# microsoft/VidTok

Hardware: AMD Instinct MI355X
Metric: encode+decode frames/sec, vidtok_kl_causal_488_4chn 17x256x256 (higher is better)
Workload: dtype bf16; 1 GPU; vidtok_kl_causal_488_4chn forward (encode+KL+decode), bf16, B=4 clips/GPU, 17x256x256; global_batch=4, launch=hipGraph replay (engine graph cache)

## Files before the change

vidtok_amd/csrc/options.cpp:

```cpp
#include "options.h"

#include <stdlib.h>
#include <string.h>

#include <atomic>
#include <mutex>

#include "../../include/vidtok_amd.h"

void vt_set_error(const char* fmt, ...);

namespace {
struct OptDef {
  const char* name;
  int dflt;
};
const OptDef kDefs[OPT_COUNT] = {
    {"conv_buf", 1},        {"conv_tinner", 1},     {"conv_ldsepi", 1},      {"conv_ws", 2},
    {"conv_narrow", 1},     {"conv_tile", 0},       {"conv_tile_min", 128},  {"conv_fuse_ln", 1}, {"conv_fuse_ln256", 1},
    {"tblock_fused", 1},    {"tblock_prof_mode", 0},
    {"conv_deep", 1},       {"ws_prof_mode", 0},    {"attn_flash", 1},      {"conv_splitk", 1},
    {"conv_tskip", 1},      {"conv_in8", 1},        {"conv_tup_ln", 1},     {"conv_nt_mb", 64},
};
std::atomic<int> g_val[OPT_COUNT];
std::once_flag g_once;

int env_default(int id) {
  char var[64] = "VT_";
  size_t n = 3;
  for (const char* s = kDefs[id].name; *s && n + 1 < sizeof(var); ++s) var[n++] = (*s >= 'a' && *s <= 'z') ? (char)(*s - 32) : *s;
  var[n] = 0;
  const char* e = getenv(var);
  return e ? atoi(e) : kDefs[id].dflt;
}
void init_all() {
  for (int i = 0; i < OPT_COUNT; ++i) g_val[i].store(env_default(i), std::memory_order_relaxed);
}
int find(const char* name) {
  if (!name) return -1;
  for (int i = 0; i < OPT_COUNT; ++i)
    if (strcmp(name, kDefs[i].name) == 0) return i;
  return -1;
}
}

int vt_opt(int id) {
  std::call_once(g_once, init_all);
  return g_val[id].load(std::memory_order_relaxed);
}

extern "C" int vt_set_option(const char* name, int32_t value) {
  const int id = find(name);
  if (id < 0) {
    vt_set_error("vt_set_option: unknown option '%s'", name ? name : "(null)");
    return VT_ERR_ARG;
  }
  std::call_once(g_once, init_all);
  g_val[id].store(value, std::memory_order_relaxed);
  return VT_OK;
}

extern "C" int vt_get_option(const char* name, int32_t* value) {
  const int id = find(name);
  if (id < 0 || !value) {
    vt_set_error("vt_get_option: unknown option '%s' or null output", name ? name : "(null)");
    return VT_ERR_ARG;
  }
  *value = vt_opt(id);
  return VT_OK;
}

extern "C" int vt_reset_options(void) {
  std::call_once(g_once, init_all);
  init_all();
  return VT_OK;
}

extern "C" int vt_option_count(void) { return OPT_COUNT; }
extern "C" const char* vt_option_name(int32_t i) { return (i >= 0 && i < OPT_COUNT) ? kDefs[i].name : nullptr; }
```

vidtok_amd/csrc/options.h:

```cpp
#pragma once

enum VtOpt {
  OPT_CONV_BUF = 0,
  OPT_CONV_TINNER,
  OPT_CONV_LDSEPI,
  OPT_CONV_WS,
  OPT_CONV_NARROW,
  OPT_CONV_TILE,
  OPT_CONV_TILE_MIN,
  OPT_CONV_FUSE_LN,
  OPT_CONV_FUSE_LN256,
  OPT_TBLOCK_FUSED,
  OPT_TBLOCK_PROF_MODE,
  OPT_CONV_DEEP,
  OPT_WS_PROF_MODE,
  OPT_ATTN_FLASH,
  OPT_CONV_SPLITK,
  OPT_CONV_TSKIP,
  OPT_CONV_IN8,
  OPT_CONV_TUP_LN,
  OPT_CONV_NT_MB,
  OPT_COUNT
};

int vt_opt(int id);
```

vidtok_amd/csrc/tblock_ws128.hip:

```cpp
#include <atomic>
#include <type_traits>

#include "conv_common.h"

#define VT_STORE_AUX 2

namespace {

[[maybe_unused]] constexpr int TB_PIX = 64;
[[maybe_unused]] constexpr int TB_ROWP = 272;
[[maybe_unused]] constexpr int TB_SLOT = TB_PIX * TB_ROWP;
[[maybe_unused]] constexpr int TB_RING = 3 * TB_SLOT;
[[maybe_unused]] constexpr int TB_T = TB_PIX * 128 * 4;

typedef uint16_t tb_h;
struct TBlockArgs {
  const tb_h* x;
  tb_h* y;
  tb_h* n_out;
  const tb_h* w1;
  const tb_h* w2;
  const float* b1;
  const float* b2;
  const float* g1; const float* be1;
  const float* g2; const float* be2;
  const float* gn; const float* ben;
  int B, T, HW;
  int replicate;
  tb_h* cache1;
  tb_h* cache2;
  int cache_off;
  int keep_y;
  int ln_next;
  float eps;
  unsigned long long* prof;
  int prof_mode;
};

template <int I, int N, typename F>
__device__ __forceinline__ void tb_static_for(F&& f) {
  if constexpr (I < N) {
    f(std::integral_constant<int, I>{});
    tb_static_for<I + 1, N>(f);
  }
}

#pragma clang fp contract(off)
typedef float f32x2 __attribute__((ext_vector_type(2)));
template <typename H>
__device__ __forceinline__ uint32_t tb_pack2(f32x2 v) {
  return h16<H>::pack(v[0], v[1]);
}

[[maybe_unused]] constexpr int T3_T1P = 256;
[[maybe_unused]] constexpr int T3_OFF_T1 = 2 * TB_RING;
[[maybe_unused]] constexpr int T3_OFF_T2 = 2 * TB_RING + TB_PIX * T3_T1P;
[[maybe_unused]] constexpr int T3_LDS = T3_OFF_T2 + TB_T;
template <typename H>
__device__ __forceinline__ void t3_unpack8(const u32x4& w, float (&v)[8]) {
#pragma unroll
  for (int q = 0; q < 4; ++q) {
    v[2 * q] = h16<H>::lo(w[q]);
    v[2 * q + 1] = h16<H>::hi(w[q]);
  }
}
template <typename H>
__device__ __forceinline__ u32x4 t3_pack8(const float (&o)[8]) {
  u32x4 w;
#pragma unroll
  for (int q = 0; q < 4; ++q) w[q] = tb_pack2<H>(f32x2{o[2 * q], o[2 * q + 1]});
  return w;
}

[[maybe_unused]] constexpr int T4_OFF_PRM = T3_LDS;
[[maybe_unused]] constexpr int T4_LDS = T4_OFF_PRM + 8 * 128 * 4;
[[maybe_unused]] constexpr int T4_FD = 6;

template <typename H, bool FIRST>
__device__ __forceinline__ void t4_mfma(const u32x4& w, const u32x4& x, f32x16& acc) {
  if constexpr (std::is_same<H, bf16_t>::value) {
    if constexpr (FIRST) asm volatile("v_mfma_f32_32x32x16_bf16 %0, %1, %2, 0" : "=v"(acc) : "a"(w), "v"(x));
    else asm volatile("v_mfma_f32_32x32x16_bf16 %0, %1, %2, %0" : "+v"(acc) : "a"(w), "v"(x));
  } else {
    if constexpr (FIRST) asm volatile("v_mfma_f32_32x32x16_f16 %0, %1, %2, 0" : "=v"(acc) : "a"(w), "v"(x));
    else asm volatile("v_mfma_f32_32x32x16_f16 %0, %1, %2, %0" : "+v"(acc) : "a"(w), "v"(x));
  }
}
template <bool SILU>
__device__ __forceinline__ void t4_row_norm(float (&v)[8], const float (&g)[8], const float (&b)[8], float eps, float (&o)[8]) {
  ln_row8<16, SILU>(v, g, b, eps, o);
}

template <typename H, int LNN, bool KEEP, bool CACHE, bool PROF = false>
__global__ __launch_bounds__(512, 1) void tblock_pair_kernel(const TBlockArgs p) {
#if defined(__HIP_DEVICE_COMPILE__)
  extern __shared__ __attribute__((aligned(16))) char smem[];
  const int tid = threadIdx.x;
  const int lane = tid & 63;
  const int wave = __builtin_amdgcn_readfirstlane(tid >> 6);
  const int cw = wave & 3, grp = wave >> 2;
  const int ptiles = p.HW / TB_PIX;
  const int ncols = p.B * ptiles;
  const int G = gridDim.x;
  const int slot_id = xcd_remap(blockIdx.x, G);
  const int cq = ncols / G, cr = ncols - cq * G;
  const int c_begin = slot_id * cq + min(slot_id, cr);
  const int c_end = c_begin + cq + (slot_id < cr ? 1 : 0);
  if (c_begin >= c_end) return;
  if (grp == 1) __builtin_amdgcn_s_setprio(2);
  const int n = (c_end - c_begin) * p.T;
  constexpr int R1 = 0, R2 = TB_RING;
  const unsigned frame_bytes = (unsigned)p.HW * 256u;

  float* prm = reinterpret_cast<float*>(smem + T4_OFF_PRM);
  {
    const int c = tid & 127, a = tid >> 7;
    const int pc = ((c >> 2) & 1) * 64 + (c >> 3) * 4 + (c & 3);
    const float* src0 = a == 0 ? p.g1 : (a == 1 ? p.be1 : (a == 2 ? p.g2 : p.be2));
    prm[a * 128 + pc] = ln_fold(src0[c], true);
    float v;
    if (a == 0) v = LNN ? ln_fold(p.gn[c], LNN == 2) : 1.0f;
    else if (a == 1) v = LNN ? ln_fold(p.ben[c], LNN == 2) : 0.0f;
    else if (a == 2) v = p.b1 ? p.b1[c] : 0.0f;
    else v = p.b2 ? p.b2[c] : 0.0f;
    prm[(a + 4) * 128 + pc] = v;
  }

  struct Cur {
    int b, pt, t;
  };
  auto cur_at = [&](int k) __attribute__((always_inline)) {
    Cur c;
    const int q = k / p.T;
    c.t = k - q * p.T;
    const int col = c_begin + q;
    c.b = col / ptiles;
    c.pt = col - c.b * ptiles;
    return c;
  };
  auto cur_step = [&](Cur& c) __attribute__((always_inline)) {
    c.t += 1;
    if (c.t == p.T) {
      c.t = 0;
      c.pt += 1;
      if (c.pt == ptiles) {
        c.pt = 0;
        c.b += 1;
      }
    }
  };
  auto frame_rsrc = [&](const tb_h* base, const Cur& c) __attribute__((always_inline)) {
    return __builtin_amdgcn_make_buffer_rsrc(const_cast<tb_h*>(base) + ((long long)c.b * p.T + c.t) * p.HW * 128, 0, frame_bytes, 0x00020000);
  };

  unsigned long long* stamps = reinterpret_cast<unsigned long long*>(smem + T4_LDS);
  int kcur = 0;
  auto stamp = [&](int i) __attribute__((always_inline)) {
    if constexpr (PROF) {
      if (blockIdx.x == 0 && kcur >= 8 && kcur < 12) {
        const unsigned long long ts = __builtin_amdgcn_s_memtime();
        if (lane == 0) stamps[((kcur - 8) * 8 + wave) * 8 + i] = ts;
      }
    }
  };
  auto dump = [&]() __attribute__((always_inline)) {
    if constexpr (PROF) {
      if (blockIdx.x == 0 && lane == 0)
        for (int i = 0; i < 32; ++i) p.prof[wave * 32 + i] = stamps[((i / 8) * 8 + wave) * 8 + (i % 8)];
    }
  };

  u32x4 wreg[24];
  {
    const tb_h* wsrc = grp == 0 ? p.w1 : p.w2;
    const long long roff = (long long)(cw * 32 + (lane & 31)) * 384 + (lane >> 5) * 8;
#pragma unroll
    for (int g = 0; g < 24; ++g) wreg[g] = *reinterpret_cast<const u32x4*>(wsrc + roff + g * 16);
    __builtin_amdgcn_s_waitcnt(0x0F70);
  }
  f32x16 acc[2];
  auto gemm = [&](auto kt0_c, int roff, int s3, int t) __attribute__((always_inline)) {
    constexpr int KT0 = decltype(kt0_c)::value;
    constexpr int M0 = 16 * KT0;
    int lo = lane;
    asm volatile("" : "+v"(lo));
    const int frag_off = roff + (lo & 31) * TB_ROWP + (lo >> 5) * 16;
    int sp[3];
#pragma unroll
    for (int kt = 0; kt < 3; ++kt) {
      const int back = (t - 2 + kt >= 0 || (CACHE && p.replicate == 2)) ? 2 - kt : t;
      int sl = s3 - back;
      sl = sl < 0 ? sl + 3 : sl;
      sp[kt] = frag_off + sl * TB_SLOT;
    }
    auto faddr = [&](int m) __attribute__((always_inline)) -> const u32x4* {
      const int g = m >> 1, j = m & 1;
      return reinterpret_cast<const u32x4*>(smem + sp[g >> 3] + j * (32 * TB_ROWP) + (g & 7) * 32);
    };
    u32x4 xf[T4_FD + 1];
#pragma unroll
    for (int m = M0; m < M0 + T4_FD; ++m) xf[m % (T4_FD + 1)] = *faddr(m);
    if (grp == 1) __builtin_amdgcn_s_setprio(3);
    tb_static_for<M0, 48>([&](auto mc) __attribute__((always_inline)) {
      constexpr int m = decltype(mc)::value;
      t4_mfma<H, (m < M0 + 2)>(wreg[m >> 1], xf[m % (T4_FD + 1)], acc[m & 1]);
      if constexpr (m + T4_FD < 48) xf[(m + T4_FD) % (T4_FD + 1)] = *faddr(m + T4_FD);
      __builtin_amdgcn_sched_barrier(0);
    });
    if (grp == 1) __builtin_amdgcn_s_setprio(2);
    asm volatile("s_nop 15\n\ts_nop 3" ::: "memory");
  };
  auto run_gemm = [&](int roff, int s3, int t) __attribute__((always_inline)) {
    const int first = p.replicate != 0 ? 0 : max(0, 2 - t);
    if (first == 0) gemm(std::integral_constant<int, 0>{}, roff, s3, t);
    else if (first == 1) gemm(std::integral_constant<int, 1>{}, roff, s3, t);
    else gemm(std::integral_constant<int, 2>{}, roff, s3, t);
  };
  auto acc_to_T1 = [&]() __attribute__((always_inline)) {
    int lo = lane;
    asm volatile("" : "+v"(lo));
    const int l31 = lo & 31;
    const int base = T3_OFF_T1 + l31 * T3_T1P + 8 * (lo >> 5);
#pragma unroll
    for (int j = 0; j < 2; ++j)
#pragma unroll
      for (int g = 0; g < 4; ++g) {
        u32x2 w;
        w[0] = tb_pack2<H>(f32x2{acc[j][4 * g], acc[j][4 * g + 1]});
        w[1] = tb_pack2<H>(f32x2{acc[j][4 * g + 2], acc[j][4 * g + 3]});
        *reinterpret_cast<u32x2*>(smem + base + j * (32 * T3_T1P) + (((4 * cw + g) ^ (l31 & 15)) << 4)) = w;
      }
  };
  auto acc_to_T2 = [&]() __attribute__((always_inline)) {
    int lo = lane;
    asm volatile("" : "+v"(lo));
    const int l31 = lo & 31;
    const int base = T3_OFF_T2 + l31 * 512 + (((cw * 8 + (lo >> 5)) ^ l31) << 4);
#pragma unroll
    for (int j = 0; j < 2; ++j)
#pragma unroll
      for (int g = 0; g < 4; ++g) {
        f32x4 v;
#pragma unroll
        for (int e = 0; e < 4; ++e) v[e] = acc[j][4 * g + e];
        *reinterpret_cast<f32x4*>(smem + ((base ^ (g << 5)) + j * (32 * 512))) = v;
      }
  };

  auto unit_geom = [&](int& oct_j, int& row0) __attribute__((always_inline)) {
    int tt = tid;
    asm volatile("" : "+v"(tt));
    const int vt = tt & 255;
    oct_j = vt & 15;
    row0 = vt >> 4;
  };
  auto ld_prm = [&](int arr, int oct_j, float (&o)[8]) __attribute__((always_inline)) {
    const f32x4 a = *reinterpret_cast<const f32x4*>(prm + arr * 128 + 4 * oct_j);
    const f32x4 b = *reinterpret_cast<const f32x4*>(prm + arr * 128 + 64 + 4 * oct_j);
#pragma unroll
    for (int e = 0; e < 4; ++e) {
      o[e] = a[e];
      o[4 + e] = b[e];
    }
  };
  auto load_rows = [&](auto u0_c, auto u1_c, u32x4 (&dst)[4], const Cur& c) __attribute__((always_inline)) {
    constexpr int U0 = decltype(u0_c)::value, U1 = decltype(u1_c)::value;
    int oct_j, row0;
    unit_geom(oct_j, row0);
    const __amdgpu_buffer_rsrc_t rs = frame_rsrc(p.x, c);
    const int vo = (c.pt * TB_PIX + row0) * 256 + oct_j * 16;
#pragma unroll
    for (int it = U0; it < U1; ++it) dst[it] = __builtin_amdgcn_raw_buffer_load_b128(rs, vo + it * (16 * 256), 0, 0);
  };
  auto cache_put = [&](tb_h* cache, const Cur& c, int oct_j, int row, const u32x4& w) __attribute__((always_inline)) {
    if constexpr (!CACHE) return;
    const int j = c.t - (p.T - p.cache_off - 2);
    if (cache != nullptr && (j == 0 || j == 1)) {
      const __amdgpu_buffer_rsrc_t rs = __builtin_amdgcn_make_buffer_rsrc(cache + ((long long)c.b * 2 + j) * p.HW * 128, 0, frame_bytes, 0x00020000);
      __builtin_amdgcn_raw_buffer_store_b128(w, rs, (c.pt * TB_PIX + row) * 256 + oct_j * 16, 0, 0);
    }
  };
  auto cache_get = [&](const tb_h* cache, int roff, const Cur& c, int sl2, int sl1) __attribute__((always_inline)) {
    if constexpr (!CACHE) return;
    int oct_j, row0;
    unit_geom(oct_j, row0);
    u32x4 w[2][4];
#pragma unroll
    for (int j = 0; j < 2; ++j) {
      const __amdgpu_buffer_rsrc_t rs = __builtin_amdgcn_make_buffer_rsrc(const_cast<tb_h*>(cache) + ((long long)c.b * 2 + j) * p.HW * 128, 0, frame_bytes, 0x00020000);
#pragma unroll
      for (int it = 0; it < 4; ++it) w[j][it] = __builtin_amdgcn_raw_buffer_load_b128(rs, (c.pt * TB_PIX + row0 + 16 * it) * 256 + oct_j * 16, 0, 0);
    }
#pragma unroll
    for (int j = 0; j < 2; ++j)
#pragma unroll
      for (int it = 0; it < 4; ++it)
        *reinterpret_cast<u32x4*>(smem + roff + (j == 0 ? sl2 : sl1) * TB_SLOT + (row0 + 16 * it) * TB_ROWP + oct_j * 16) = w[j][it];
  };
  auto ln1_units = [&](auto u0_c, auto u1_c, const u32x4 (&xr)[4], int s3, const Cur& c) __attribute__((always_inline)) {
    constexpr int U0 = decltype(u0_c)::value, U1 = decltype(u1_c)::value;
    int oct_j, row0;
    unit_geom(oct_j, row0);
    float g[8], b[8];
    ld_prm(0, oct_j, g);
    ld_prm(1, oct_j, b);
    const int wo = R1 + s3 * TB_SLOT + row0 * TB_ROWP + oct_j * 16;
#pragma unroll
    for (int it = U0; it < U1; ++it) {
      float v[8], o[8];
      t3_unpack8<H>(xr[it], v);
      t4_row_norm<true>(v, g, b, p.eps, o);
      const u32x4 w = t3_pack8<H>(o);
      *reinterpret_cast<u32x4*>(smem + wo + it * (16 * TB_ROWP)) = w;
      cache_put(p.cache1, c, oct_j, row0 + 16 * it, w);
      __builtin_amdgcn_sched_barrier(0);
    }
  };

  auto out_store = [&](const u32x4& w, __amdgpu_buffer_rsrc_t rs, int vo) __attribute__((always_inline)) {
    if constexpr (PROF) {
      if (p.prof_mode & 16) return;
    }
    __builtin_amdgcn_raw_buffer_store_b128(w, rs, vo, 0, VT_STORE_AUX);
  };
  struct XSet {
    u32x4 xn[4], xr[4];
  };
  XSet xs;
  Cur c_p2 = cur_at(0);
  Cur c_p1 = c_p2, c_0 = c_p2, c_m1 = c_p2, c_m2 = c_p2;
  __syncthreads();
  constexpr int L1G0 = 3;
  using IL = std::integral_constant<int, L1G0>;
  if (grp == 0) {
    load_rows(std::integral_constant<int, 0>{}, IL{}, xs.xn, c_0);
    ln1_units(std::integral_constant<int, 0>{}, IL{}, xs.xn, 0, c_0);
  } else {
    load_rows(IL{}, std::integral_constant<int, 4>{}, xs.xn, c_0);
    ln1_units(IL{}, std::integral_constant<int, 4>{}, xs.xn, 0, c_0);
    if (CACHE && p.replicate == 2) cache_get(p.cache1, R1, c_0, 1, 2);
  }
  cur_step(c_p1);
  c_p2 = c_p1;
  cur_step(c_p2);
  if (1 < n) {
    if (grp == 0) load_rows(std::integral_constant<int, 0>{}, IL{}, xs.xn, c_p1);
    else load_rows(IL{}, std::integral_constant<int, 4>{}, xs.xn, c_p1);
  }
  if (grp == 0) {
#pragma unroll
    for (int it = 0; it < 2; ++it) xs.xr[it] = xs.xn[0];
  } else {
#pragma unroll
    for (int it = 2; it < 4; ++it) xs.xr[it] = xs.xn[3];
  }
  int s3 = 0;
  auto advance = [&]() __attribute__((always_inline)) {
    c_m2 = c_m1;
    c_m1 = c_0;
    c_0 = c_p1;
    c_p1 = c_p2;
    cur_step(c_p2);
    s3 = s3 == 2 ? 0 : s3 + 1;
  };
  auto slot_back = [&](int back) __attribute__((always_inline)) {
    const int s = s3 - back;
    return s < 0 ? s + 3 : s;
  };
  __syncthreads();

  auto l2_units = [&](auto u0_c, auto u1_c, int sl, const Cur& c) __attribute__((always_inline)) {
    constexpr int U0 = decltype(u0_c)::value, U1 = decltype(u1_c)::value;
    int oct_j, row0;
    unit_geom(oct_j, row0);
    float bo1[8], g[8], b[8];
    ld_prm(6, oct_j, bo1);
    ld_prm(2, oct_j, g);
    ld_prm(3, oct_j, b);
    const int ro = T3_OFF_T1 + row0 * T3_T1P + ((oct_j ^ row0) << 4);
    const int wo = R2 + sl * TB_SLOT + row0 * TB_ROWP + oct_j * 16;
    u32x4 tw[4];
    tw[U0] = *reinterpret_cast<const u32x4*>(smem + ro + U0 * (16 * T3_T1P));
#pragma unroll
    for (int it = U0; it < U1; ++it) {
      if (it + 1 < U1) tw[it + 1] = *reinterpret_cast<const u32x4*>(smem + ro + (it + 1) * (16 * T3_T1P));
      float v[8], o[8];
      t3_unpack8<H>(tw[it], v);
#pragma unroll
      for (int e = 0; e < 8; ++e) v[e] = v[e] + bo1[e];
      t4_row_norm<true>(v, g, b, p.eps, o);
      const u32x4 w = t3_pack8<H>(o);
      *reinterpret_cast<u32x4*>(smem + wo + it * (16 * TB_ROWP)) = w;
      cache_put(p.cache2, c, oct_j, row0 + 16 * it, w);
      __builtin_amdgcn_sched_barrier(0);
    }
  };
  auto o_unit = [&](auto it_c, const u32x4& xrow, const Cur& c) __attribute__((always_inline)) {
    constexpr int it = decltype(it_c)::value;
    int oct_j, row0;
    unit_geom(oct_j, row0);
    float bo2[8], gn[8], bn[8];
    ld_prm(7, oct_j, bo2);
    if constexpr (LNN != 0) {
      ld_prm(4, oct_j, gn);
      ld_prm(5, oct_j, bn);
    }
    const int vo = (c.pt * TB_PIX + row0) * 256 + oct_j * 16 + it * (16 * 256);
    const int tb = T3_OFF_T2 + row0 * 512 + (((2 * oct_j) ^ row0) << 4);
    const int to = ((it & 1) ? (tb ^ 256) : tb) + it * (16 * 512);
    const f32x4 t0 = *reinterpret_cast<const f32x4*>(smem + to);
    const f32x4 t1 = *reinterpret_cast<const f32x4*>(smem + (to ^ 16));
    float v[8], xv[8];
    t3_unpack8<H>(xrow, xv);
#pragma unroll
    for (int e = 0; e < 8; ++e) v[e] = xv[e] + ((e < 4 ? t0[e] : t1[e - 4]) + bo2[e]);
    if constexpr (KEEP) out_store(t3_pack8<H>(v), frame_rsrc(p.y, c), vo);
    if constexpr (LNN != 0) {
      float o[8];
      t4_row_norm<(LNN == 2)>(v, gn, bn, p.eps, o);
      out_store(t3_pack8<H>(o), frame_rsrc(p.n_out, c), vo);
    }
    __builtin_amdgcn_sched_barrier(0);
  };
  using I0 = std::integral_constant<int, 0>;
  using I1 = std::integral_constant<int, 1>;
  using I2 = std::integral_constant<int, 2>;
  using I3 = std::integral_constant<int, 3>;
  using I4 = std::integral_constant<int, 4>;

  if (grp == 0) {
    auto body = [&](auto guard_c, int k) __attribute__((always_inline)) {
      constexpr bool GUARD = decltype(guard_c)::value;
      kcur = k;
      stamp(0);
      if ((!GUARD || k < n) && !(PROF && (p.prof_mode & 1))) run_gemm(R1, s3, c_0.t);
      stamp(1);
      if ((!GUARD || (k >= 1 && k - 1 < n)) && !(PROF && (p.prof_mode & 2))) l2_units(I3{}, I4{}, slot_back(1), c_m1);
      if (CACHE && p.replicate == 2 && k >= 1 && k - 1 < n && c_m1.t == 0) cache_get(p.cache2, R2, c_m1, s3, slot_back(2));
      stamp(2);
      __syncthreads();
      if (!GUARD || k < n) acc_to_T1();
      stamp(3);
      const bool do_o = (!GUARD || (k >= 2 && k - 2 < n)) && !(PROF && (p.prof_mode & 2));
      const bool do_l1 = (!GUARD || k + 1 < n) && !(PROF && (p.prof_mode & 2));
      const bool ld_r = !GUARD || (k >= 1 && k - 1 < n);
      const bool ld_n = !GUARD || k + 2 < n;
      if (do_o) o_unit(I0{}, xs.xr[0], c_m2);
      if (ld_r) load_rows(I0{}, I1{}, xs.xr, c_m1);
      if (do_l1) ln1_units(I0{}, I1{}, xs.xn, slot_back(2), c_p1);
      if (ld_n) load_rows(I0{}, I1{}, xs.xn, c_p2);
      if (do_o) o_unit(I1{}, xs.xr[1], c_m2);
      if (ld_r) load_rows(I1{}, I2{}, xs.xr, c_m1);
      stamp(4);
      if (do_l1) ln1_units(I1{}, IL{}, xs.xn, slot_back(2), c_p1);
      if (ld_n) load_rows(I1{}, IL{}, xs.xn, c_p2);
      stamp(5);
      __syncthreads();
      stamp(6);
      advance();
    };
    int k = 0;
    for (; k < 2 && k < n + 2; ++k) body(std::true_type{}, k);
    __builtin_amdgcn_s_waitcnt(0x0F70);
    for (; k + 2 < n; ++k) body(std::false_type{}, k);
    for (; k < n + 2; ++k) body(std::true_type{}, k);
  } else {
    auto body = [&](auto guard_c, int k) __attribute__((always_inline)) {
      constexpr bool GUARD = decltype(guard_c)::value;
      kcur = k;
      stamp(0);
      if (!GUARD || (k >= 2 && k - 2 < n)) acc_to_T2();
      stamp(1);
      if ((!GUARD || (k >= 1 && k - 1 < n)) && !(PROF && (p.prof_mode & 2))) l2_units(I0{}, I3{}, slot_back(1), c_m1);
      stamp(2);
      __syncthreads();
      if ((!GUARD || (k >= 1 && k - 1 < n)) && !(PROF && (p.prof_mode & 1))) run_gemm(R2, slot_back(1), c_m1.t);
      stamp(3);
      const bool do_o = (!GUARD || (k >= 2 && k - 2 < n)) && !(PROF && (p.prof_mode & 2));
      const bool do_l1 = (!GUARD || k + 1 < n) && !(PROF && (p.prof_mode & 2));
      const bool ld_r = !GUARD || (k >= 1 && k - 1 < n);
      const bool ld_n = !GUARD || k + 2 < n;
      if (do_o) o_unit(I2{}, xs.xr[2], c_m2);
      if (ld_r) load_rows(I2{}, I3{}, xs.xr, c_m1);
      stamp(4);
      if (do_l1) ln1_units(IL{}, I4{}, xs.xn, slot_back(2), c_p1);
      if (ld_n) load_rows(IL{}, I4{}, xs.xn, c_p2);
      if (do_o) o_unit(I3{}, xs.xr[3], c_m2);
      if (ld_r) load_rows(I3{}, I4{}, xs.xr, c_m1);
      if (CACHE && p.replicate == 2 && k + 1 < n && c_p1.t == 0) cache_get(p.cache1, R1, c_p1, slot_back(1), s3);
      stamp(5);
      __syncthreads();
      stamp(6);
      advance();
    };
    int k = 0;
    for (; k < 2 && k < n + 2; ++k) body(std::true_type{}, k);
    __builtin_amdgcn_s_waitcnt(0x0F70);
    for (; k + 2 < n; ++k) body(std::false_type{}, k);
    for (; k < n + 2; ++k) body(std::true_type{}, k);
  }
  dump();
#endif
}

}

extern "C" int vt_tblock_desc_size(void) { return (int)sizeof(vt_tblock_desc); }

extern "C" int vt_temporal_block_supported(const vt_tblock_desc* d) {
  if (!d) return 0;
  if (!vt_is_h16(d->dtype) || d->C != 128 || d->ld != 128) return 0;
  if (d->B <= 0 || d->T <= 0 || d->HW <= 0 || d->HW % TB_PIX != 0) return 0;
  if (d->tmode != VT_TPAD_ZERO && d->tmode != VT_TPAD_REPLICATE && d->tmode != VT_TPAD_CACHE) return 0;
  if (d->tmode == VT_TPAD_CACHE && (d->cache1 == nullptr || d->cache2 == nullptr)) return 0;
  if ((d->cache1 != nullptr || d->cache2 != nullptr) && (d->cache_offset < 0 || d->T - d->cache_offset < 3)) return 0;
  if (d->ln_next_mode < 0 || d->ln_next_mode > 2) return 0;
  if (vt_opt(OPT_TBLOCK_FUSED) == 0) return 0;
  return 1;
}

namespace {
int tblock_launch(const vt_tblock_desc* d, vt_stream stream_, unsigned long long* prof) {
  hipStream_t stream = reinterpret_cast<hipStream_t>(stream_);
  VT_CHECK_ARG(d != nullptr, "vt_temporal_block: null descriptor");
  VT_CHECK_ARG(vt_temporal_block_supported(d),
               "vt_temporal_block: only bf16 / fp16, C = ld = 128, HW %% 64 == 0; cache mode needs both caches, kept chunk state "
               "T - cache_offset >= 3 (got dtype %d C %d ld %d HW %lld T %d tmode %d cache_offset %d)", d->dtype, d->C, d->ld,
               (long long)d->HW, d->T, d->tmode, d->cache_offset);
  VT_CHECK_ARG(d->x && d->w1 && d->w2 && d->norm1_gamma && d->norm1_beta && d->norm2_gamma && d->norm2_beta,
               "vt_temporal_block: null tensor pointer");
  VT_CHECK_ARG(d->keep_y || d->ln_next_mode != 0, "vt_temporal_block: nothing to write (keep_y = 0 and no next norm)");
  VT_CHECK_ARG(!d->keep_y || d->y, "vt_temporal_block: y is null");
  VT_CHECK_ARG(d->ln_next_mode == 0 || (d->next_gamma && d->next_beta && d->n_out), "vt_temporal_block: next norm needs gamma, beta, n_out");
  const uintptr_t al = reinterpret_cast<uintptr_t>(d->x) | reinterpret_cast<uintptr_t>(d->y) | reinterpret_cast<uintptr_t>(d->n_out) |
                       reinterpret_cast<uintptr_t>(d->w1) | reinterpret_cast<uintptr_t>(d->w2);
  VT_CHECK_ARG((al & 15) == 0, "vt_temporal_block: tensors must be 16-byte aligned");
  TBlockArgs a;
  a.x = (const tb_h*)d->x; a.y = (tb_h*)d->y; a.n_out = (tb_h*)d->n_out;
  a.w1 = (const tb_h*)d->w1; a.w2 = (const tb_h*)d->w2; a.b1 = d->b1; a.b2 = d->b2;
  a.g1 = d->norm1_gamma; a.be1 = d->norm1_beta; a.g2 = d->norm2_gamma; a.be2 = d->norm2_beta;
  a.gn = d->next_gamma; a.ben = d->next_beta;
  a.B = d->B; a.T = d->T; a.HW = (int)d->HW;
  a.replicate = d->tmode == VT_TPAD_REPLICATE ? 1 : (d->tmode == VT_TPAD_CACHE ? 2 : 0);
  a.cache1 = (tb_h*)d->cache1; a.cache2 = (tb_h*)d->cache2; a.cache_off = d->cache_offset;
  VT_CHECK_ARG(((reinterpret_cast<uintptr_t>(d->cache1) | reinterpret_cast<uintptr_t>(d->cache2)) & 15) == 0, "vt_temporal_block: caches must be 16-byte aligned");
  a.keep_y = d->keep_y ? 1 : 0;
  a.ln_next = d->ln_next_mode;
  a.eps = d->eps;
  a.prof = prof;
  a.prof_mode = prof ? vt_opt(OPT_TBLOCK_PROF_MODE) : 0;
  VT_CHECK_ARG((long long)d->HW * 256 < (1ll << 31), "vt_temporal_block: frames of at most 2^23 pixels");
#define VT_TB_KERNS(H)                                                                                                              \
  reinterpret_cast<const void*>(&tblock_pair_kernel<H, 0, true, false>), reinterpret_cast<const void*>(&tblock_pair_kernel<H, 1, true, false>),      \
      reinterpret_cast<const void*>(&tblock_pair_kernel<H, 1, false, false>), reinterpret_cast<const void*>(&tblock_pair_kernel<H, 2, true, false>), \
      reinterpret_cast<const void*>(&tblock_pair_kernel<H, 2, false, false>), reinterpret_cast<const void*>(&tblock_pair_kernel<H, 0, true, true>),  \
      reinterpret_cast<const void*>(&tblock_pair_kernel<H, 1, true, true>), reinterpret_cast<const void*>(&tblock_pair_kernel<H, 1, false, true>),   \
      reinterpret_cast<const void*>(&tblock_pair_kernel<H, 2, true, true>), reinterpret_cast<const void*>(&tblock_pair_kernel<H, 2, false, true>)
  constexpr int NK = 21;
  static const void* const kerns2[NK] = {VT_TB_KERNS(bf16_t), VT_TB_KERNS(f16_t), reinterpret_cast<const void*>(&tblock_pair_kernel<bf16_t, 2, true, false, true>)};
#undef VT_TB_KERNS
  const bool cached = a.replicate == 2 || a.cache1 != nullptr || a.cache2 != nullptr;
  int ki = a.ln_next == 0 ? 0 : (a.ln_next == 1 ? (a.keep_y ? 1 : 2) : (a.keep_y ? 3 : 4));
  int lds = T4_LDS;
  const unsigned threads = 512;
  if (cached) ki += 5;
  if (d->dtype == VT_F16) ki += 10;
  if (prof != nullptr) {
    VT_CHECK_ARG(d->dtype == VT_BF16 && a.ln_next == 2 && a.keep_y && !cached, "vt_temporal_block_profile: bf16, ln_next_mode 2 and keep_y only, no chunk state");
    ki = 20;
    lds += 2048;
  }
  const void* kern = kerns2[ki];
  static std::atomic<bool> attr_done[NK][kMaxDevices];
  for (int k = 0; k < NK; ++k)
    if (const int rc = vt_dynamic_lds(kerns2[k], k == 20 ? T4_LDS + 2048 : T4_LDS, attr_done[k])) return rc;
  const int ncu = device_cus();
  const long long ncols = (long long)d->B * (d->HW / TB_PIX);
  const int grid = ncols < ncu ? (int)ncols : ncu;
  void* kargs[] = {&a};
  VT_CHECK_HIP(hipLaunchKernel(kern, dim3((unsigned)grid), dim3(threads), kargs, lds, stream));
  return VT_OK;
}
}

extern "C" int vt_temporal_block(const vt_tblock_desc* d, vt_stream stream) { return tblock_launch(d, stream, nullptr); }

extern "C" int vt_temporal_block_profile(const vt_tblock_desc* d, uint64_t* stamps_out, vt_stream stream) {
  VT_CHECK_ARG(stamps_out != nullptr, "vt_temporal_block_profile: null output");
  return tblock_launch(d, stream, reinterpret_cast<unsigned long long*>(stamps_out));
}
```

Before: 938.8 frames/s.

## Add 12-wave temporal block kernel with dedicated load/output wave group

Adds a 12-wave variant of the fused temporal block kernel and makes it the default. A third wave group takes over input row loads, LN1 prologue, the residual output and next-layer norm, so the two GEMM groups mostly just run MFMAs and the epilogues. Because of register pressure at 768 threads, weights now feed MFMA from VGPRs instead of AGPRs and the fragment prefetch depth is reduced. Extra waves can add scheduling overlap but also register spills and more barrier participants.

```diff
diff --git a/vidtok_amd/csrc/options.cpp b/vidtok_amd/csrc/options.cpp
--- a/vidtok_amd/csrc/options.cpp
+++ b/vidtok_amd/csrc/options.cpp
@@ -21,6 +21,7 @@
     {"tblock_fused", 1},    {"tblock_prof_mode", 0},
     {"conv_deep", 1},       {"ws_prof_mode", 0},    {"attn_flash", 1},      {"conv_splitk", 1},
     {"conv_tskip", 1},      {"conv_in8", 1},        {"conv_tup_ln", 1},     {"conv_nt_mb", 64},
+    {"tblock_waves", 12},
 };
 std::atomic<int> g_val[OPT_COUNT];
 std::once_flag g_once;
diff --git a/vidtok_amd/csrc/options.h b/vidtok_amd/csrc/options.h
--- a/vidtok_amd/csrc/options.h
+++ b/vidtok_amd/csrc/options.h
@@ -20,6 +20,7 @@
   OPT_CONV_IN8,
   OPT_CONV_TUP_LN,
   OPT_CONV_NT_MB,
+  OPT_TBLOCK_WAVES,
   OPT_COUNT
 };
 
diff --git a/vidtok_amd/csrc/tblock_ws128.hip b/vidtok_amd/csrc/tblock_ws128.hip
--- a/vidtok_amd/csrc/tblock_ws128.hip
+++ b/vidtok_amd/csrc/tblock_ws128.hip
@@ -75,10 +75,19 @@
 [[maybe_unused]] constexpr int T4_OFF_PRM = T3_LDS;
 [[maybe_unused]] constexpr int T4_LDS = T4_OFF_PRM + 8 * 128 * 4;
 [[maybe_unused]] constexpr int T4_FD = 6;
-
-template <typename H, bool FIRST>
+[[maybe_unused]] constexpr int T4_FD12 = 4;
+
+template <typename H, bool FIRST, bool WA = true>
 __device__ __forceinline__ void t4_mfma(const u32x4& w, const u32x4& x, f32x16& acc) {
-  if constexpr (std::is_same<H, bf16_t>::value) {
+  if constexpr (!WA) {
+    if constexpr (std::is_same<H, bf16_t>::value) {
+      if constexpr (FIRST) asm volatile("v_mfma_f32_32x32x16_bf16 %0, %1, %2, 0" : "=v"(acc) : "v"(w), "v"(x));
+      else asm volatile("v_mfma_f32_32x32x16_bf16 %0, %1, %2, %0" : "+v"(acc) : "v"(w), "v"(x));
+    } else {
+      if constexpr (FIRST) asm volatile("v_mfma_f32_32x32x16_f16 %0, %1, %2, 0" : "=v"(acc) : "v"(w), "v"(x));
+      else asm volatile("v_mfma_f32_32x32x16_f16 %0, %1, %2, %0" : "+v"(acc) : "v"(w), "v"(x));
+    }
+  } else if constexpr (std::is_same<H, bf16_t>::value) {
     if constexpr (FIRST) asm volatile("v_mfma_f32_32x32x16_bf16 %0, %1, %2, 0" : "=v"(acc) : "a"(w), "v"(x));
     else asm volatile("v_mfma_f32_32x32x16_bf16 %0, %1, %2, %0" : "+v"(acc) : "a"(w), "v"(x));
   } else {
@@ -91,8 +100,8 @@
   ln_row8<16, SILU>(v, g, b, eps, o);
 }
 
-template <typename H, int LNN, bool KEEP, bool CACHE, bool PROF = false>
-__global__ __launch_bounds__(512, 1) void tblock_pair_kernel(const TBlockArgs p) {
+template <typename H, int LNN, bool KEEP, bool CACHE, int NW = 8, bool PROF = false>
+__global__ __launch_bounds__(NW * 64, 1) void tblock_pair_kernel(const TBlockArgs p) {
 #if defined(__HIP_DEVICE_COMPILE__)
   extern __shared__ __attribute__((aligned(16))) char smem[];
   const int tid = threadIdx.x;
@@ -108,12 +117,13 @@
   const int c_end = c_begin + cq + (slot_id < cr ? 1 : 0);
   if (c_begin >= c_end) return;
   if (grp == 1) __builtin_amdgcn_s_setprio(2);
+  if (NW == 12 && grp == 2) __builtin_amdgcn_s_setprio(1);
   const int n = (c_end - c_begin) * p.T;
   constexpr int R1 = 0, R2 = TB_RING;
   const unsigned frame_bytes = (unsigned)p.HW * 256u;
 
   float* prm = reinterpret_cast<float*>(smem + T4_OFF_PRM);
-  {
+  if (tid < 512) {
     const int c = tid & 127, a = tid >> 7;
     const int pc = ((c >> 2) & 1) * 64 + (c >> 3) * 4 + (c & 3);
     const float* src0 = a == 0 ? p.g1 : (a == 1 ? p.be1 : (a == 2 ? p.g2 : p.be2));
@@ -159,25 +169,26 @@
     if constexpr (PROF) {
       if (blockIdx.x == 0 && kcur >= 8 && kcur < 12) {
         const unsigned long long ts = __builtin_amdgcn_s_memtime();
-        if (lane == 0) stamps[((kcur - 8) * 8 + wave) * 8 + i] = ts;
+        if (lane == 0) stamps[((kcur - 8) * NW + wave) * 8 + i] = ts;
       }
     }
   };
   auto dump = [&]() __attribute__((always_inline)) {
     if constexpr (PROF) {
       if (blockIdx.x == 0 && lane == 0)
-        for (int i = 0; i < 32; ++i) p.prof[wave * 32 + i] = stamps[((i / 8) * 8 + wave) * 8 + (i % 8)];
+        for (int i = 0; i < 32; ++i) p.prof[wave * 32 + i] = stamps[((i / 8) * NW + wave) * 8 + (i % 8)];
     }
   };
 
   u32x4 wreg[24];
-  {
+  auto load_weights = [&]() __attribute__((always_inline)) {
     const tb_h* wsrc = grp == 0 ? p.w1 : p.w2;
     const long long roff = (long long)(cw * 32 + (lane & 31)) * 384 + (lane >> 5) * 8;
 #pragma unroll
     for (int g = 0; g < 24; ++g) wreg[g] = *reinterpret_cast<const u32x4*>(wsrc + roff + g * 16);
     __builtin_amdgcn_s_waitcnt(0x0F70);
-  }
+  };
+  if constexpr (NW == 8) load_weights();
   f32x16 acc[2];
   auto gemm = [&](auto kt0_c, int roff, int s3, int t) __attribute__((always_inline)) {
     constexpr int KT0 = decltype(kt0_c)::value;
@@ -197,14 +208,15 @@
       const int g = m >> 1, j = m & 1;
       return reinterpret_cast<const u32x4*>(smem + sp[g >> 3] + j * (32 * TB_ROWP) + (g & 7) * 32);
     };
-    u32x4 xf[T4_FD + 1];
-#pragma unroll
-    for (int m = M0; m < M0 + T4_FD; ++m) xf[m % (T4_FD + 1)] = *faddr(m);
+    constexpr int FD = NW == 12 ? T4_FD12 : T4_FD;
+    u32x4 xf[FD + 1];
+#pragma unroll
+    for (int m = M0; m < M0 + FD; ++m) xf[m % (FD + 1)] = *faddr(m);
     if (grp == 1) __builtin_amdgcn_s_setprio(3);
     tb_static_for<M0, 48>([&](auto mc) __attribute__((always_inline)) {
       constexpr int m = decltype(mc)::value;
-      t4_mfma<H, (m < M0 + 2)>(wreg[m >> 1], xf[m % (T4_FD + 1)], acc[m & 1]);
-      if constexpr (m + T4_FD < 48) xf[(m + T4_FD) % (T4_FD + 1)] = *faddr(m + T4_FD);
+      t4_mfma<H, (m < M0 + 2), NW == 8>(wreg[m >> 1], xf[m % (FD + 1)], acc[m & 1]);
+      if constexpr (m + FD < 48) xf[(m + FD) % (FD + 1)] = *faddr(m + FD);
       __builtin_amdgcn_sched_barrier(0);
     });
     if (grp == 1) __builtin_amdgcn_s_setprio(2);
@@ -328,11 +340,18 @@
   };
   XSet xs;
   Cur c_p2 = cur_at(0);
-  Cur c_p1 = c_p2, c_0 = c_p2, c_m1 = c_p2, c_m2 = c_p2;
+  Cur c_p1 = c_p2, c_0 = c_p2, c_m1 = c_p2, c_m2 = c_p2, c_m3 = c_p2;
   __syncthreads();
   constexpr int L1G0 = 3;
   using IL = std::integral_constant<int, L1G0>;
-  if (grp == 0) {
+  if constexpr (NW == 12) {
+    if (grp == 2) {
+      load_rows(std::integral_constant<int, 0>{}, std::integral_constant<int, 4>{}, xs.xn, c_0);
+      ln1_units(std::integral_constant<int, 0>{}, std::integral_constant<int, 4>{}, xs.xn, 0, c_0);
+    } else if (grp == 1) {
+      if (CACHE && p.replicate == 2) cache_get(p.cache1, R1, c_0, 1, 2);
+    }
+  } else if (grp == 0) {
     load_rows(std::integral_constant<int, 0>{}, IL{}, xs.xn, c_0);
     ln1_units(std::integral_constant<int, 0>{}, IL{}, xs.xn, 0, c_0);
   } else {
@@ -344,10 +363,17 @@
   c_p2 = c_p1;
   cur_step(c_p2);
   if (1 < n) {
-    if (grp == 0) load_rows(std::integral_constant<int, 0>{}, IL{}, xs.xn, c_p1);
+    if constexpr (NW == 12) {
+      if (grp == 2) load_rows(std::integral_constant<int, 0>{}, std::integral_constant<int, 2>{}, xs.xn, c_p1);
+    } else if (grp == 0) load_rows(std::integral_constant<int, 0>{}, IL{}, xs.xn, c_p1);
     else load_rows(IL{}, std::integral_constant<int, 4>{}, xs.xn, c_p1);
   }
-  if (grp == 0) {
+  if constexpr (NW == 12) {
+    if (grp == 2) {
+#pragma unroll
+      for (int it = 0; it < 4; ++it) xs.xr[it] = xs.xn[it];
+    }
+  } else if (grp == 0) {
 #pragma unroll
     for (int it = 0; it < 2; ++it) xs.xr[it] = xs.xn[0];
   } else {
@@ -356,6 +382,7 @@
   }
   int s3 = 0;
   auto advance = [&]() __attribute__((always_inline)) {
+    if constexpr (NW == 12) c_m3 = c_m2;
     c_m2 = c_m1;
     c_m1 = c_0;
     c_0 = c_p1;
@@ -374,20 +401,28 @@
     int oct_j, row0;
     unit_geom(oct_j, row0);
     float bo1[8], g[8], b[8];
-    ld_prm(6, oct_j, bo1);
-    ld_prm(2, oct_j, g);
-    ld_prm(3, oct_j, b);
+    if constexpr (NW == 8) {
+      ld_prm(6, oct_j, bo1);
+      ld_prm(2, oct_j, g);
+      ld_prm(3, oct_j, b);
+    }
     const int ro = T3_OFF_T1 + row0 * T3_T1P + ((oct_j ^ row0) << 4);
     const int wo = R2 + sl * TB_SLOT + row0 * TB_ROWP + oct_j * 16;
     u32x4 tw[4];
-    tw[U0] = *reinterpret_cast<const u32x4*>(smem + ro + U0 * (16 * T3_T1P));
+    if constexpr (NW == 8) tw[U0] = *reinterpret_cast<const u32x4*>(smem + ro + U0 * (16 * T3_T1P));
 #pragma unroll
     for (int it = U0; it < U1; ++it) {
-      if (it + 1 < U1) tw[it + 1] = *reinterpret_cast<const u32x4*>(smem + ro + (it + 1) * (16 * T3_T1P));
+      if constexpr (NW == 12) tw[it] = *reinterpret_cast<const u32x4*>(smem + ro + it * (16 * T3_T1P));
+      else if (it + 1 < U1) tw[it + 1] = *reinterpret_cast<const u32x4*>(smem + ro + (it + 1) * (16 * T3_T1P));
       float v[8], o[8];
       t3_unpack8<H>(tw[it], v);
+      if constexpr (NW == 12) ld_prm(6, oct_j, bo1);
 #pragma unroll
       for (int e = 0; e < 8; ++e) v[e] = v[e] + bo1[e];
+      if constexpr (NW == 12) {
+        ld_prm(2, oct_j, g);
+        ld_prm(3, oct_j, b);
+      }
       t4_row_norm<true>(v, g, b, p.eps, o);
       const u32x4 w = t3_pack8<H>(o);
       *reinterpret_cast<u32x4*>(smem + wo + it * (16 * TB_ROWP)) = w;
@@ -422,12 +457,47 @@
     }
     __builtin_amdgcn_sched_barrier(0);
   };
+  auto o_head = [&](auto it_c, const u32x4& xrow, const Cur& c, float (&v)[8]) __attribute__((always_inline)) {
+    constexpr int it = decltype(it_c)::value;
+    int oct_j, row0;
+    unit_geom(oct_j, row0);
+    float bo2[8];
+    ld_prm(7, oct_j, bo2);
+    const int vo = (c.pt * TB_PIX + row0) * 256 + oct_j * 16 + it * (16 * 256);
+    const int tb = T3_OFF_T2 + row0 * 512 + (((2 * oct_j) ^ row0) << 4);
+    const int to = ((it & 1) ? (tb ^ 256) : tb) + it * (16 * 512);
+    const f32x4 t0 = *reinterpret_cast<const f32x4*>(smem + to);
+    const f32x4 t1 = *reinterpret_cast<const f32x4*>(smem + (to ^ 16));
+    float xv[8];
+    t3_unpack8<H>(xrow, xv);
+#pragma unroll
+    for (int e = 0; e < 8; ++e) v[e] = xv[e] + ((e < 4 ? t0[e] : t1[e - 4]) + bo2[e]);
+    if constexpr (KEEP) out_store(t3_pack8<H>(v), frame_rsrc(p.y, c), vo);
+    __builtin_amdgcn_sched_barrier(0);
+  };
+  auto o_tail = [&](auto it_c, const float (&v)[8], const Cur& c) __attribute__((always_inline)) {
+    constexpr int it = decltype(it_c)::value;
+    if constexpr (LNN != 0) {
+      int oct_j, row0;
+      unit_geom(oct_j, row0);
+      float gn[8], bn[8], vv[8], o[8];
+      ld_prm(4, oct_j, gn);
+      ld_prm(5, oct_j, bn);
+#pragma unroll
+      for (int e = 0; e < 8; ++e) vv[e] = v[e];
+      const int vo = (c.pt * TB_PIX + row0) * 256 + oct_j * 16 + it * (16 * 256);
+      t4_row_norm<(LNN == 2)>(vv, gn, bn, p.eps, o);
+      out_store(t3_pack8<H>(o), frame_rsrc(p.n_out, c), vo);
+      __builtin_amdgcn_sched_barrier(0);
+    }
+  };
   using I0 = std::integral_constant<int, 0>;
   using I1 = std::integral_constant<int, 1>;
   using I2 = std::integral_constant<int, 2>;
   using I3 = std::integral_constant<int, 3>;
   using I4 = std::integral_constant<int, 4>;
 
+  if constexpr (NW == 8) {
   if (grp == 0) {
     auto body = [&](auto guard_c, int k) __attribute__((always_inline)) {
       constexpr bool GUARD = decltype(guard_c)::value;
@@ -499,6 +569,111 @@
     for (; k + 2 < n; ++k) body(std::false_type{}, k);
     for (; k < n + 2; ++k) body(std::true_type{}, k);
   }
+  } else {
+    constexpr int TAIL_B = 0;
+    if (grp == 0) {
+      load_weights();
+      auto body = [&](auto guard_c, int k) __attribute__((always_inline)) {
+        constexpr bool GUARD = decltype(guard_c)::value;
+        kcur = k;
+        stamp(0);
+        stamp(1);
+        if ((!GUARD || k < n) && !(PROF && (p.prof_mode & 1))) run_gemm(R1, s3, c_0.t);
+        stamp(2);
+        __syncthreads();
+        const bool do_l1 = (!GUARD || k + 1 < n) && !(PROF && (p.prof_mode & 2));
+        if (do_l1) {
+          u32x4 xg[4];
+          load_rows(I2{}, I4{}, xg, c_p1);
+          if (!GUARD || k < n) acc_to_T1();
+          stamp(3);
+          ln1_units(I2{}, I4{}, xg, slot_back(2), c_p1);
+        } else {
+          if (!GUARD || k < n) acc_to_T1();
+          stamp(3);
+        }
+        if (CACHE && p.replicate == 2 && k + 1 < n && c_p1.t == 0) cache_get(p.cache1, R1, c_p1, slot_back(1), s3);
+        stamp(4);
+        stamp(5);
+        __syncthreads();
+        stamp(6);
+        advance();
+      };
+      int k = 0;
+      for (; k < 2 && k < n + 2; ++k) body(std::true_type{}, k);
+      for (; k + 2 < n; ++k) body(std::false_type{}, k);
+      for (; k < n + 2; ++k) body(std::true_type{}, k);
+    } else if (grp == 1) {
+      load_weights();
+      auto body = [&](auto guard_c, int k) __attribute__((always_inline)) {
+        constexpr bool GUARD = decltype(guard_c)::value;
+        kcur = k;
+        stamp(0);
+        if (!GUARD || (k >= 2 && k - 2 < n)) acc_to_T2();
+        stamp(1);
+        if ((!GUARD || (k >= 1 && k - 1 < n)) && !(PROF && (p.prof_mode & 2))) l2_units(I0{}, I4{}, slot_back(1), c_m1);
+        stamp(2);
+        __syncthreads();
+        if ((!GUARD || (k >= 1 && k - 1 < n)) && !(PROF && (p.prof_mode & 1))) run_gemm(R2, slot_back(1), c_m1.t);
+        stamp(3);
+        stamp(4);
+        stamp(5);
+        __syncthreads();
+        stamp(6);
+        advance();
+      };
+      int k = 0;
+      for (; k < 2 && k < n + 2; ++k) body(std::true_type{}, k);
+      for (; k + 2 < n; ++k) body(std::false_type{}, k);
+      for (; k < n + 2; ++k) body(std::true_type{}, k);
+    } else {
+      float ov[4][8];
+#pragma unroll
+      for (int it = 0; it < 4; ++it)
+#pragma unroll
+        for (int e = 0; e < 8; ++e) ov[it][e] = 0.0f;
+      auto body = [&](auto guard_c, int k) __attribute__((always_inline)) {
+        constexpr bool GUARD = decltype(guard_c)::value;
+        kcur = k;
+        stamp(0);
+        const bool do_t = (!GUARD || (k >= 3 && k - 3 < n)) && !(PROF && (p.prof_mode & 2));
+        if (do_t) tb_static_for<TAIL_B, 4>([&](auto it_c) __attribute__((always_inline)) { o_tail(it_c, ov[decltype(it_c)::value], c_m3); });
+        stamp(1);
+        if (CACHE && p.replicate == 2 && k >= 1 && k - 1 < n && c_m1.t == 0) cache_get(p.cache2, R2, c_m1, s3, slot_back(2));
+        stamp(2);
+        __syncthreads();
+        stamp(3);
+        const bool do_o = (!GUARD || (k >= 2 && k - 2 < n)) && !(PROF && (p.prof_mode & 2));
+        const bool do_l1 = (!GUARD || k + 1 < n) && !(PROF && (p.prof_mode & 2));
+        const bool ld_r = !GUARD || (k >= 1 && k - 1 < n);
+        const bool ld_n = !GUARD || k + 2 < n;
+        tb_static_for<0, 4>([&](auto it_c) __attribute__((always_inline)) {
+          constexpr int it = decltype(it_c)::value;
+          using IN = std::integral_constant<int, it + 1>;
+          if (do_o) {
+            o_head(it_c, xs.xr[it], c_m2, ov[it]);
+            if constexpr (it < TAIL_B) o_tail(it_c, ov[it], c_m2);
+          }
+          if (ld_r) load_rows(it_c, IN{}, xs.xr, c_m1);
+          if constexpr (it < 2) {
+            if (do_l1) ln1_units(it_c, IN{}, xs.xn, slot_back(2), c_p1);
+            if (ld_n) load_rows(it_c, IN{}, xs.xn, c_p2);
+          }
+          if constexpr (it == 1) stamp(4);
+        });
+        stamp(5);
+        __syncthreads();
+        stamp(6);
+        advance();
+      };
+      int k = 0;
+      for (; k < 3 && k < n + 2; ++k) body(std::true_type{}, k);
+      __builtin_amdgcn_s_waitcnt(0x0F70);
+      for (; k + 2 < n; ++k) body(std::false_type{}, k);
+      for (; k < n + 2; ++k) body(std::true_type{}, k);
+      if (!(PROF && (p.prof_mode & 2))) tb_static_for<TAIL_B, 4>([&](auto it_c) __attribute__((always_inline)) { o_tail(it_c, ov[decltype(it_c)::value], c_m3); });
+    }
+  }
   dump();
 #endif
 }
@@ -550,30 +725,33 @@
   a.prof = prof;
   a.prof_mode = prof ? vt_opt(OPT_TBLOCK_PROF_MODE) : 0;
   VT_CHECK_ARG((long long)d->HW * 256 < (1ll << 31), "vt_temporal_block: frames of at most 2^23 pixels");
-#define VT_TB_KERNS(H)                                                                                                              \
-  reinterpret_cast<const void*>(&tblock_pair_kernel<H, 0, true, false>), reinterpret_cast<const void*>(&tblock_pair_kernel<H, 1, true, false>),      \
-      reinterpret_cast<const void*>(&tblock_pair_kernel<H, 1, false, false>), reinterpret_cast<const void*>(&tblock_pair_kernel<H, 2, true, false>), \
-      reinterpret_cast<const void*>(&tblock_pair_kernel<H, 2, false, false>), reinterpret_cast<const void*>(&tblock_pair_kernel<H, 0, true, true>),  \
-      reinterpret_cast<const void*>(&tblock_pair_kernel<H, 1, true, true>), reinterpret_cast<const void*>(&tblock_pair_kernel<H, 1, false, true>),   \
-      reinterpret_cast<const void*>(&tblock_pair_kernel<H, 2, true, true>), reinterpret_cast<const void*>(&tblock_pair_kernel<H, 2, false, true>)
-  constexpr int NK = 21;
-  static const void* const kerns2[NK] = {VT_TB_KERNS(bf16_t), VT_TB_KERNS(f16_t), reinterpret_cast<const void*>(&tblock_pair_kernel<bf16_t, 2, true, false, true>)};
+#define VT_TB_KERNS(H, NW)                                                                                                              \
+  reinterpret_cast<const void*>(&tblock_pair_kernel<H, 0, true, false, NW>), reinterpret_cast<const void*>(&tblock_pair_kernel<H, 1, true, false, NW>),      \
+      reinterpret_cast<const void*>(&tblock_pair_kernel<H, 1, false, false, NW>), reinterpret_cast<const void*>(&tblock_pair_kernel<H, 2, true, false, NW>), \
+      reinterpret_cast<const void*>(&tblock_pair_kernel<H, 2, false, false, NW>), reinterpret_cast<const void*>(&tblock_pair_kernel<H, 0, true, true, NW>),  \
+      reinterpret_cast<const void*>(&tblock_pair_kernel<H, 1, true, true, NW>), reinterpret_cast<const void*>(&tblock_pair_kernel<H, 1, false, true, NW>),   \
+      reinterpret_cast<const void*>(&tblock_pair_kernel<H, 2, true, true, NW>), reinterpret_cast<const void*>(&tblock_pair_kernel<H, 2, false, true, NW>)
+  constexpr int NK1 = 21, NK = 2 * NK1;
+  static const void* const kerns2[NK] = {VT_TB_KERNS(bf16_t, 8),  VT_TB_KERNS(f16_t, 8),  reinterpret_cast<const void*>(&tblock_pair_kernel<bf16_t, 2, true, false, 8, true>),
+                                         VT_TB_KERNS(bf16_t, 12), VT_TB_KERNS(f16_t, 12), reinterpret_cast<const void*>(&tblock_pair_kernel<bf16_t, 2, true, false, 12, true>)};
 #undef VT_TB_KERNS
   const bool cached = a.replicate == 2 || a.cache1 != nullptr || a.cache2 != nullptr;
   int ki = a.ln_next == 0 ? 0 : (a.ln_next == 1 ? (a.keep_y ? 1 : 2) : (a.keep_y ? 3 : 4));
   int lds = T4_LDS;
-  const unsigned threads = 512;
+  const int nw = vt_opt(OPT_TBLOCK_WAVES) == 8 ? 8 : 12;
+  const unsigned threads = 64u * nw;
   if (cached) ki += 5;
   if (d->dtype == VT_F16) ki += 10;
   if (prof != nullptr) {
     VT_CHECK_ARG(d->dtype == VT_BF16 && a.ln_next == 2 && a.keep_y && !cached, "vt_temporal_block_profile: bf16, ln_next_mode 2 and keep_y only, no chunk state");
     ki = 20;
-    lds += 2048;
-  }
+    lds += 256 * nw;
+  }
+  if (nw == 12) ki += NK1;
   const void* kern = kerns2[ki];
   static std::atomic<bool> attr_done[NK][kMaxDevices];
   for (int k = 0; k < NK; ++k)
-    if (const int rc = vt_dynamic_lds(kerns2[k], k == 20 ? T4_LDS + 2048 : T4_LDS, attr_done[k])) return rc;
+    if (const int rc = vt_dynamic_lds(kerns2[k], k % NK1 == 20 ? T4_LDS + 256 * (k < NK1 ? 8 : 12) : T4_LDS, attr_done[k])) return rc;
   const int ncu = device_cus();
   const long long ncols = (long long)d->B * (d->HW / TB_PIX);
   const int grid = ncols < ncu ? (int)ncols : ncu;
```

Result: no change. 942.0 frames/s (median of 6 runs) (+0.3%).
